# blindopen/TSM-Det-Pointcloud-

Measured on AMD Instinct MI355X. Metric: point-cloud frames/sec (fwd+bwd), higher is better.
Workload: dtype f32; 1 GPU; BASELINE configs[1]: KITTI-shaped synthetic, 20000 pts / 16000 active voxels per frame, full SECOND detector (VoxelBackBone8x) fwd+bwd+AdamW step; batch_per_gpu=4, global_batch=4, parallelism=dp1, voxelize_on_gpu=True

## Files before the change

include/spx.h:

```cpp
#ifndef SPX_H_
#define SPX_H_

#include <stddef.h>
#include <stdint.h>

#ifdef __cplusplus
extern "C" {
#endif

#define SPX_ABI_VERSION 3

#define SPX_OK 0
#define SPX_ERR_INVALID_ARG (-1)
#define SPX_ERR_WORKSPACE (-2)
#define SPX_ERR_UNSUPPORTED (-3)
#define SPX_ERR_LAUNCH (-4)
#define SPX_ERR_TOO_LARGE (-5)
#define SPX_ERR_CAPACITY (-7)
#define SPX_ERR_TABLE_FULL (-6)
#define SPX_ERR_RING_STALL (-8)
#define SPX_ERR_BATCH_STATS (-10)
#define SPX_ERR_OUT_OF_GRID (-9)

#define SPX_WS_PRECLEARED 1
// ... 112 lines not shown

int spx_bn_add_relu_fwd(const float *x, const float *res, int64_t n, const int64_t *d_n, int c, const float *gamma,
                        const float *beta, float *running_mean, float *running_var, int64_t *num_batches_tracked,
                        float momentum, float eps, int relu, float *y, int64_t y_ld, float *save_mean, float *save_invstd,
                        void *ws, size_t ws_bytes, spx_stream_t stream);
int spx_bn_add_relu_bwd(const float *x, const float *res, const float *dy, int64_t dy_ld, int64_t n, const int64_t *d_n,
                        int c, const float *gamma, const float *beta, const float *save_mean, const float *save_invstd, int relu,
                        float *dx, float *dres, float *dgamma, float *dbeta, void *ws, size_t ws_bytes,
                        spx_stream_t stream);

int spx_bn_apply(const float *x, const float *res, int64_t n, const int64_t *d_n, int c, const float *mean,
                 const float *invstd, const float *gamma, const float *beta, int relu, float *y, int64_t y_ld,
                 spx_stream_t stream);

int spx_bn_relu_fwd_from_sums(const float *x, int64_t n, const int64_t *d_n, int c, const float *partial, int64_t nblk,
                              const float *gamma,
                              const float *beta, float *running_mean, float *running_var, int64_t *num_batches_tracked,
                              float momentum, float eps, int relu, float *y, int64_t y_ld, float *save_mean,
                              float *save_invstd, spx_stream_t stream);

int64_t spx_wino_stat_rows(int32_t n, int32_t h, int32_t w);
int64_t spx_wino_weight_floats(int32_t cin, int32_t cout);
int spx_wino_weight(const float *w, int64_t s_o, int64_t s_i, int64_t s_a, int64_t s_b, int32_t cin, int32_t cout, int flip,
                    float *u, spx_stream_t stream);
int spx_conv2d_wino(const float *x, int64_t x_ld, const float *u, int32_t n, int32_t h, int32_t w, int32_t cin, int32_t cout,
                    const float *scale, const float *shift, int relu, float *y, int64_t y_ld, float *stat_partials,
                    spx_stream_t stream);

size_t spx_wino_wgrad_ws_bytes(int32_t cin, int32_t cout);
int spx_conv2d_wino_wgrad(const float *x, int64_t x_ld, const float *dy, int64_t dy_ld, int32_t n, int32_t h, int32_t w,
                          int32_t cin, int32_t cout, float *dw, int64_t s_o, int64_t s_i, int64_t s_a, int64_t s_b, void *ws,
                          size_t ws_bytes, spx_stream_t stream);

int spx_voxel_query(const float *new_xyz, const float *xyz, const int32_t *new_coords, const int32_t *point_indices,
                    int64_t m, int batch, const int32_t *shape3, int nsample, float radius, const int32_t *range3,
                    int32_t *idx, int32_t *cnt_unique, spx_stream_t stream);

int spx_voxel_query_dilated(const float *new_xyz, const float *xyz, const int32_t *new_coords,
                            const int32_t *point_indices, int64_t m, int batch, const int32_t *shape3, int nsample,
                            float former_radius, float radius, const int32_t *range3, const int32_t *stride3,
                            int32_t *idx, int32_t *cnt_unique, int32_t *idx_cnt, spx_stream_t stream);


size_t spx_furthest_point_sample_ws_bytes(int32_t b, int64_t n);
int spx_furthest_point_sample(const float *xyz, const float *weights, int32_t b, int64_t n, int32_t npoint, int32_t *idx,
                              void *ws, size_t ws_bytes, spx_stream_t stream);

size_t spx_furthest_point_sample_matrix_ws_bytes(int32_t b, int64_t n);
int spx_furthest_point_sample_matrix(const float *matrix, const float *weights, int32_t b, int64_t n, int32_t npoint,
                                     int32_t *idx, void *ws, size_t ws_bytes, spx_stream_t stream);

int spx_ball_query(const float *xyz, const float *new_xyz, int32_t b, int64_t n, int64_t m, float r_in, float r_out,
                   int32_t nsample, int32_t *idx_cnt, int32_t *idx, spx_stream_t stream);

int spx_group_points(const float *features, const int32_t *idx, int32_t b, int32_t c, int64_t n, int64_t m,
                     int32_t nsample, float *out, spx_stream_t stream);

size_t spx_group_points_bwd_ws_bytes(int32_t b, int64_t n, int64_t m, int32_t nsample);
int spx_group_points_bwd(const float *grad_out, const int32_t *idx, int32_t b, int32_t c, int64_t n, int64_t m,
                         int32_t nsample, float *grad_features, void *ws, size_t ws_bytes, spx_stream_t stream);

int spx_three_nn(const float *unknown, const float *known, int32_t b, int64_t n, int64_t m, float *dist2, int32_t *idx,
                 spx_stream_t stream);

int spx_three_interpolate(const float *features, const int32_t *idx, const float *weight, int32_t b, int32_t c, int64_t m,
                          int64_t n, float *out, spx_stream_t stream);
// ... 210 lines not shown
```

tsm-det-pointcloud-_amd/pcdet_amd/models/dense_heads/anchor_head_single.py:

```python
import os

import numpy as np
import torch
import torch.nn as nn
import torch.nn.functional as F

from ..model_utils import det_wgrad
from .anchor_head_template import AnchorHeadTemplate


_HYBRID = os.environ.get("SPX_HEAD_HYBRID", "1") != "0"


class _PointwiseHeadsFn(torch.autograd.Function):

    @staticmethod
    def forward(ctx, x, w, b):
        ctx.save_for_backward(x, w)
        return F.linear(x.permute(0, 2, 3, 1), w.flatten(1), b)

    @staticmethod
    def backward(ctx, dy):
        x, w = ctx.saved_tensors
        dy = dy.contiguous()
        n, h, wd, co = dy.shape
        dx = (dy.view(-1, co) @ w.flatten(1)).view(n, h, wd, x.shape[1]).permute(0, 3, 1, 2)
        if not dy.is_cuda:
            _, dw, db = torch.ops.aten.convolution_backward(dy.permute(0, 3, 1, 2), x, w, [co], [1, 1], [0, 0], [1, 1],
                                                            False, [0, 0], 1, [False, True, True])
            return dx, dw, db
        dw, db = det_wgrad.pointwise_wgrad(dy.view(-1, co), x.permute(0, 2, 3, 1).reshape(-1, x.shape[1]))
        return dx, dw.view_as(w), db


class AnchorHeadSingle(AnchorHeadTemplate):
    def __init__(self, model_cfg, input_channels, num_class, class_names, grid_size, point_cloud_range,
                 predict_boxes_when_training=True, **kwargs):
        super().__init__(model_cfg=model_cfg, num_class=num_class, class_names=class_names, grid_size=grid_size,
                         point_cloud_range=point_cloud_range, predict_boxes_when_training=predict_boxes_when_training)
        self.num_anchors_per_location = sum(self.num_anchors_per_location)
        self.conv_cls = nn.Conv2d(input_channels, self.num_anchors_per_location * self.num_class, kernel_size=1)
        self.conv_box = nn.Conv2d(input_channels, self.num_anchors_per_location * self.box_coder.code_size,
                                  kernel_size=1)
        if self.model_cfg.get('USE_DIRECTION_CLASSIFIER', None) is not None:
            self.conv_dir_cls = nn.Conv2d(input_channels, self.num_anchors_per_location * self.model_cfg.NUM_DIR_BINS,
                                          kernel_size=1)
        else:
            self.conv_dir_cls = None
        self.init_weights()

    def init_weights(self):
        pi = 0.01
        nn.init.constant_(self.conv_cls.bias, -np.log((1 - pi) / pi))
        nn.init.normal_(self.conv_box.weight, mean=0, std=0.001)

    def _heads(self, x):
        convs = [self.conv_cls, self.conv_box] + ([self.conv_dir_cls] if self.conv_dir_cls is not None else [])
        w = torch.cat([c.weight for c in convs], 0)
        b = torch.cat([c.bias for c in convs], 0)
        if (not x.is_contiguous(memory_format=torch.channels_last) or torch.is_autocast_enabled()
                or (torch.is_grad_enabled() and not _HYBRID)):
            y = F.conv2d(x, w, b).permute(0, 2, 3, 1)
        elif not torch.is_grad_enabled():
            y = F.linear(x.permute(0, 2, 3, 1), w.flatten(1), b)
        else:
            y = _PointwiseHeadsFn.apply(x, w, b)
        outs = [t.contiguous() for t in torch.split(y, [c.out_channels for c in convs], dim=3)]
        return outs[0], outs[1], (outs[2] if len(outs) > 2 else None)

    def forward(self, data_dict):
        if data_dict.get('encoded_bev_features', None) is not None:
            feats = data_dict['encoded_bev_features']
            x = feats[0] if len(feats) == 1 else torch.cat(feats, dim=1)
        else:
            x = data_dict['spatial_features_2d']
        x = x.float()
        cls_preds, box_preds, dir_cls_preds = self._heads(x)
        self.forward_ret_dict['cls_preds'] = cls_preds
        self.forward_ret_dict['box_preds'] = box_preds
        if dir_cls_preds is not None:
            self.forward_ret_dict['dir_cls_preds'] = dir_cls_preds
        if self.training:
            self.forward_ret_dict.update(self.assign_targets(gt_boxes=data_dict['gt_boxes']))
        if not self.training or self.predict_boxes_when_training:
            batch_cls_preds, batch_box_preds = self.generate_predicted_boxes(
                batch_size=data_dict['batch_size'], cls_preds=cls_preds, box_preds=box_preds,
                dir_cls_preds=dir_cls_preds)
            data_dict['batch_cls_preds'] = batch_cls_preds
            data_dict['batch_box_preds'] = batch_box_preds
            data_dict['cls_preds_normalized'] = False
        return data_dict
```

tsm-det-pointcloud-_amd/pcdet_amd/models/model_utils/det_wgrad.py:

```python
import torch
import torch.nn.functional as F

CHUNK = 4096


def mm_fixed(at, b):
    k = at.shape[1]
    s = k // CHUNK
    if s <= 1:
        return at @ b
    kk = s * CHUNK
    parts = torch.bmm(at[:, :kk].unflatten(1, (s, CHUNK)).transpose(0, 1), b[:kk].unflatten(0, (s, CHUNK)))
    out = parts.sum(0)
    if kk < k:
        out = out + at[:, kk:] @ b[kk:]
    return out


def rows_tn(a, b):
    return mm_fixed(a.t(), b)


def _rows(t):
    return t.permute(0, 2, 3, 1).reshape(-1, t.shape[1])


class _ConvFn(torch.autograd.Function):
    @staticmethod
    def forward(ctx, x, w, stride, padding, transposed):
        ctx.save_for_backward(x, w)
        ctx.cfg = (stride, padding, transposed)
        if transposed:
            return F.conv_transpose2d(x, w, None, stride)
        return F.conv2d(x, w, None, stride, padding)

    @staticmethod
    def backward(ctx, dy):
        x, w = ctx.saved_tensors
        stride, padding, transposed = ctx.cfg
        dx = dw = None
        if ctx.needs_input_grad[0]:
            dx = torch.ops.aten.convolution_backward(dy, x, w, None, [stride] * 2, [padding] * 2, [1, 1], transposed,
                                                     [0, 0], 1, [True, False, False])[0]
        if ctx.needs_input_grad[1]:
            n = x.shape[0]
            if transposed:
                s, co = stride, w.shape[1]
                h, wd = x.shape[2], x.shape[3]
                d = dy.permute(0, 2, 3, 1).reshape(n, h, s, wd, s, co).permute(0, 1, 3, 5, 2, 4).reshape(n * h * wd, co * s * s)
                dw = rows_tn(_rows(x), d).view_as(w)
            else:
                k, co = w.shape[2], w.shape[0]
                acc = None
                for i in range(n):
                    cols = F.unfold(x[i:i + 1], k, padding=padding, stride=stride)[0]
                    part = mm_fixed(cols, dy[i].permute(1, 2, 0).reshape(-1, co))
                    acc = part if acc is None else acc + part
                dw = acc.t().reshape(w.shape)
        return dx, dw, None, None, None


def usable(x, m):
    if not (x.is_cuda and x.dtype == torch.float32 and torch.is_grad_enabled() and m.weight.requires_grad
            and m.bias is None and m.groups == 1 and tuple(m.dilation) == (1, 1) and not torch.is_autocast_enabled()):
        return False
    k, s = tuple(m.kernel_size), tuple(m.stride)
    if k[0] != k[1] or s[0] != s[1]:
        return False
    if isinstance(m, torch.nn.ConvTranspose2d):
        return k == s and tuple(m.padding) == (0, 0) and tuple(m.output_padding) == (0, 0)
    return isinstance(m, torch.nn.Conv2d)


def conv2d(x, m, padding):
    return _ConvFn.apply(x, m.weight, int(m.stride[0]), int(padding), False)


def conv_transpose2d(x, m):
    return _ConvFn.apply(x, m.weight, int(m.stride[0]), 0, True)


def pointwise_wgrad(dy_rows, x_rows):
    return rows_tn(dy_rows, x_rows), dy_rows.sum(0)
```

tsm-det-pointcloud-_amd/spx/_lib.py:

```python
import ctypes
import os

import torch

_HERE = os.path.dirname(os.path.abspath(__file__))
LIB_PATH = os.environ.get("SPX_LIB_PATH") or os.path.join(os.path.dirname(_HERE), "csrc", "libspx.so")

SPX_ABI_VERSION = 3
SPX_MAX_KVOL = 32

_vp = ctypes.c_void_p
_i64 = ctypes.c_int64
_int = ctypes.c_int
_sz = ctypes.c_size_t
_i32p = ctypes.POINTER(ctypes.c_int32)
_f32p = ctypes.POINTER(ctypes.c_float)
_vpp = ctypes.POINTER(ctypes.c_void_p)

class PointMlp(ctypes.Structure):
    _fields_ = [("w1", _vp), ("bn_mean", _vp), ("bn_var", _vp), ("bn_weight", _vp), ("bn_bias", _vp),
                ("bn_eps", ctypes.c_float), ("w2", _vp), ("b2", _vp)]


_mlpp = ctypes.POINTER(PointMlp)
# ... 32 lines not shown
    "spx_conv_ring_stat_rows": (_int, []),
    "spx_conv_ring_tiles_per_wave": (_int, [_int]),
    "spx_conv_ring_plan": (_int, [_vp, _i64, _int, _i64, _vp, _vp, _vp]),
    "spx_conv_gemm_ring": (_int, [_vp, _i64, _int, _vp, _int, _int, _int, _vp, _i64, _i64, _vp, _vp, _vp, _int, _vp, _vp, _vp,
                                  _vp, _vp, _vp]),
    "spx_conv_wgrad_ws_bytes": (_sz, [_int, _int, _int, _i64]),
    "spx_conv_wgrad_counts_bytes": (_sz, [_int, _i64]),
    "spx_conv_wgrad_counts": (_int, [_vp, _i64, _int, _i64, _vp, _vp, _vp]),
    "spx_conv_wgrad": (_int, [_vp, _int, _vp, _int, _int, _vp, _i64, _i64, _vp, _vp, _vp, _vp, _sz, _vp]),
    "spx_densify": (_int, [_vp, _vp, _i64, _vp, _int, _int, _i32p, _int, _vp, _vp]),
    "spx_densify_bwd": (_int, [_vp, _vp, _i64, _vp, _int, _int, _i32p, _int, _vp, _vp]),
    "spx_boxes_iou_bev": (_int, [_vp, _i64, _vp, _i64, _int, _vp, _vp]),
    "spx_nms_ws_bytes": (_sz, [_i64]),
    "spx_nms_bev": (_int, [_vp, _i64, ctypes.c_float, _int, _vp, _vp, _vp, _sz, _vp]),
    "spx_assign_targets_ws_bytes": (_sz, [_int, _int, _int]),
    "spx_bn_relu_ws_bytes": (_sz, [_int]),
    "spx_bn_relu_fwd": (_int, [_vp, _i64, _vp, _int, _vp, _vp, _vp, _vp, ctypes.c_float, ctypes.c_float, _int, _vp, _vp,
                               _vp, _vp, _sz, _vp]),
    "spx_bn_relu_bwd": (_int, [_vp, _vp, _i64, _vp, _int, _vp, _vp, _vp, _vp, _int, _vp, _vp, _vp, _vp, _sz, _vp]),
    "spx_bn_add_relu_fwd": (_int, [_vp, _vp, _i64, _vp, _int, _vp, _vp, _vp, _vp, _vp, ctypes.c_float, ctypes.c_float, _int,
                                   _vp, _i64, _vp, _vp, _vp, _sz, _vp]),
    "spx_bn_add_relu_bwd": (_int, [_vp, _vp, _vp, _i64, _i64, _vp, _int, _vp, _vp, _vp, _vp, _int, _vp, _vp, _vp, _vp, _vp, _sz,
                                   _vp]),
    "spx_bn_apply": (_int, [_vp, _vp, _i64, _vp, _int, _vp, _vp, _vp, _vp, _int, _vp, _i64, _vp]),
    "spx_wino_weight_floats": (_i64, [_int, _int]),
    "spx_wino_weight": (_int, [_vp, _i64, _i64, _i64, _i64, _int, _int, _int, _vp, _vp]),
    "spx_conv2d_wino": (_int, [_vp, _i64, _vp, _int, _int, _int, _int, _int, _vp, _vp, _int, _vp, _i64, _vp, _vp]),
    "spx_wino_stat_rows": (_i64, [_int, _int, _int]),
    "spx_bn_relu_fwd_from_sums": (_int, [_vp, _i64, _vp, _int, _vp, _i64, _vp, _vp, _vp, _vp, _vp, ctypes.c_float, ctypes.c_float,
                                         _int, _vp, _i64, _vp, _vp, _vp]),
    "spx_wino_wgrad_ws_bytes": (_sz, [_int, _int]),
    "spx_conv2d_wino_wgrad": (_int, [_vp, _i64, _vp, _i64, _int, _int, _int, _int, _int, _vp, _i64, _i64, _i64, _i64, _vp, _sz,
                                     _vp]),
    "spx_anchor_loss_ws_bytes": (_sz, [_int, _i64]),
    "spx_anchor_loss": (_int, [_vp, _vp, _vp, _vp, _vp, _vp, _int, _i64, _int, _int, ctypes.c_float, ctypes.c_float,
                               ctypes.c_float, ctypes.c_float, ctypes.c_float, ctypes.c_float, _vp, _vp, _vp, _vp, _vp, _sz,
                               _vp]),
    "spx_assign_targets": (_int, [_vp, _int, _i64, _int, _vp, _int, _int, _vp, _int, _vp, _vp, _vp, _vp, _vp, _vp, _sz,
                                  _vp]),
    "spx_furthest_point_sample_ws_bytes": (_sz, [ctypes.c_int32, _i64]),
    "spx_furthest_point_sample": (_int, [_vp, _vp, ctypes.c_int32, _i64, ctypes.c_int32, _vp, _vp, _sz, _vp]),
    "spx_furthest_point_sample_matrix_ws_bytes": (_sz, [ctypes.c_int32, _i64]),
    "spx_furthest_point_sample_matrix": (_int, [_vp, _vp, ctypes.c_int32, _i64, ctypes.c_int32, _vp, _vp, _sz, _vp]),
    "spx_ball_query": (_int, [_vp, _vp, ctypes.c_int32, _i64, _i64, ctypes.c_float, ctypes.c_float, ctypes.c_int32, _vp,
                              _vp, _vp]),
    "spx_group_points": (_int, [_vp, _vp, ctypes.c_int32, ctypes.c_int32, _i64, _i64, ctypes.c_int32, _vp, _vp]),
    "spx_group_points_bwd_ws_bytes": (_sz, [ctypes.c_int32, _i64, _i64, ctypes.c_int32]),
    "spx_group_points_bwd": (_int, [_vp, _vp, ctypes.c_int32, ctypes.c_int32, _i64, _i64, ctypes.c_int32, _vp, _vp, _sz,
                                    _vp]),
    "spx_three_nn": (_int, [_vp, _vp, ctypes.c_int32, _i64, _i64, _vp, _vp, _vp]),
    "spx_three_interpolate": (_int, [_vp, _vp, _vp, ctypes.c_int32, ctypes.c_int32, _i64, _i64, _vp, _vp]),
    "spx_three_interpolate_bwd_ws_bytes": (_sz, [ctypes.c_int32, _i64, _i64]),
    "spx_three_interpolate_bwd": (_int, [_vp, _vp, _vp, ctypes.c_int32, ctypes.c_int32, _i64, _i64, _vp, _vp, _sz, _vp]),
    "spx_points_in_boxes": (_int, [_vp, _vp, ctypes.c_int32, _i64, _i64, _vp, _vp]),
    "spx_roiaware_pool3d_ws_bytes": (_sz, [_i64, _i64, ctypes.c_int32, ctypes.c_int32, ctypes.c_int32]),
    "spx_roiaware_pool3d_fwd": (_int, [_vp, _vp, _vp, _i64, _i64, ctypes.c_int32, ctypes.c_int32, ctypes.c_int32,
                                       ctypes.c_int32, ctypes.c_int32, ctypes.c_int32, _vp, _vp, _vp, _vp, _vp, _sz, _vp]),
    "spx_roiaware_pool3d_bwd": (_int, [_vp, _vp, _vp, _vp, _i64, _i64, ctypes.c_int32, ctypes.c_int32, ctypes.c_int32,
                                       ctypes.c_int32, ctypes.c_int32, _vp, _vp]),
    "spx_group_project": (_int, [_vp, _vp, _vp, _vp, _vp, _vp, ctypes.c_int32, _i64, ctypes.c_int32, _i64, ctypes.c_int32,
                                 _vp, _vp]),
    "spx_group_project_bwd_ws_bytes": (_sz, [ctypes.c_int32, _i64, ctypes.c_int32, _i64, ctypes.c_int32]),
    "spx_group_project_bwd": (_int, [_vp, _vp, _vp, _vp, _vp, ctypes.c_int32, _i64, ctypes.c_int32, _i64, ctypes.c_int32,
                                     _vp, _vp, _vp, _sz, _vp]),
    "spx_point_vote": (_int, [_vp, _vp, ctypes.c_int32, ctypes.c_int32, _i64, _i64, _i64, _mlpp, ctypes.c_int32, _f32p,
                              _vp, _vp]),
# ... 114 lines not shown
```

tsm-det-pointcloud-_amd/spx/functional.py:

```python
import os
import weakref

import torch

from . import ops


def _packed(weight, mode):
    if weight.is_cuda and torch.cuda.is_current_stream_capturing():
        if not torch.is_grad_enabled():
            holder = weight._base if weight._base is not None else weight
            hit = (getattr(holder, "_spx_packed", None) or {}).get(
                (mode, weight.data_ptr(), tuple(weight.shape), tuple(weight.stride())))
            if hit is not None and hit[0] == weight._version:
                return _graph_constant(weight, hit[1], lambda w, out, mode=mode: ops.pack_weight(w, mode, out=out))
        return ops.pack_weight(weight, mode)
    holder = weight._base if weight._base is not None else weight
    cache = getattr(holder, "_spx_packed", None)
    if cache is None:
        cache = {}
        try:
            holder._spx_packed = cache
        except AttributeError:
            return ops.pack_weight(weight, mode)
# ... 99 lines not shown
    for w, (fwd, bwd) in zip(ws, bank.views):
        geom = (w.data_ptr(), tuple(w.shape), tuple(w.stride()))
        try:
            w._spx_packed = {(0,) + geom: (w._version, fwd), (1,) + geom: (w._version, bwd)}
        except AttributeError:
            pass
    return True


_ASYNC_WGRAD = os.environ.get("SPX_ASYNC_WGRAD", "1") != "0"
_DEFER_JOIN = os.environ.get("SPX_WGRAD_DEFER_JOIN", "1") != "0"
_SIDE_STREAMS = {}


def _side_stream(device):
    s = _SIDE_STREAMS.get(device.index)
    if s is None:
        s = _SIDE_STREAMS[device.index] = torch.cuda.Stream(device=device)
    return s


_DEFERRED = set()


def _join_after_backward(main, side, keep):
    def _join():
        main.wait_stream(side)
        keep.clear()
        _DEFERRED.clear()
    torch.autograd.Variable._execution_engine.queue_callback(_join)


def _off_critical_path(fn, reads, weight):
    dev = reads[0].device
    main = torch.cuda.current_stream(dev)
    side = _side_stream(dev)
    side.wait_stream(main)
    with torch.cuda.stream(side):
        g = fn()
    g.record_stream(main)
    if (_nobody_reads_before_the_optimizer(weight) and id(weight) not in _DEFERRED
            and tuple(g.shape) == tuple(weight.shape) and g.stride() == weight.stride()):
        _DEFERRED.add(id(weight))
        _join_after_backward(main, side, list(reads))
    else:
        main.wait_stream(side)
    return g


def _nobody_reads_before_the_optimizer(weight):
    if not _DEFER_JOIN or not weight.is_leaf or weight.grad is not None or torch.cuda.is_current_stream_capturing():
        return False
    if getattr(weight, "_backward_hooks", None) or getattr(weight, "_post_accumulate_grad_hooks", None):
        return False
    dist = torch.distributed
    if dist.is_available() and dist.is_initialized():
        return bool(getattr(weight, "_spx_manual_reduce", False))
    return True


def _conv(src, wp, c_dst, kvol, pair, ld, n_dst, flip, scale, shift, relu, d_n, rb, want_stats=False):
    out = stats = None
    if rb is not None and src.is_cuda and n_dst > 0 and src.shape[0] > 0:
        if ops.ring_ok(src.shape[1], c_dst, n_dst, kvol):
            perm, table, tld, plan = ops.ring_plan_for(rb, pair, ld, kvol, n_dst, d_n)
            out = ops.conv_gemm_ring(src, wp, c_dst, kvol, table, tld, n_dst, plan, flip_k=flip, scale=scale, shift=shift,
                                     relu=relu, d_n_dst=d_n, perm=perm, want_stats=want_stats)
            if want_stats:
                out, stats = out
        elif ops.balanced_ok(src.shape[1], c_dst, n_dst, rb, pair):
            if ops.grouped_ok(rb, kvol):
                perm, grouped, plan = ops.grouped_plan_for(rb, pair, ld, kvol, n_dst, d_n)
                out = ops.conv_gemm_balanced(src, wp, c_dst, kvol, grouped, n_dst, n_dst, plan, flip_k=flip, scale=scale,
                                             shift=shift, relu=relu, d_n_dst=d_n, perm=perm)
            else:
                plan = ops.plan_for(rb, pair, ld, kvol, n_dst, d_n)
                out = ops.conv_gemm_balanced(src, wp, c_dst, kvol, pair, ld, n_dst, plan, flip_k=flip, scale=scale,
                                             shift=shift, relu=relu, d_n_dst=d_n)
    if out is None:
        out = ops.conv_gemm(src, wp, c_dst, kvol, pair, ld, n_dst, flip_k=flip, scale=scale, shift=shift, relu=relu,
# ... 335 lines not shown
```

tsm-det-pointcloud-_amd/spx/ops.py:

```python
import ctypes
import os

import torch

from . import _lib
from ._lib import check, f_arr, i3

_WS = {}


_raw_stream = getattr(torch._C, "_cuda_getCurrentRawStream", None)


def _stream_handle(device):
    if _raw_stream is not None:
        idx = device.index
        return _raw_stream(torch.cuda.current_device() if idx is None else idx)
    return torch.cuda.current_stream(device).cuda_stream


def _stream(t):
    return ctypes.c_void_p(_stream_handle(t.device))


# ... 685 lines not shown
        raise ValueError("weight image does not match Cin=%d, Cout=%d" % (cin, cout))
    part = None
    if stats:
        part = torch.empty((lib.spx_wino_stat_rows(n, h, w), 2, cout), dtype=torch.float32, device=x.device)
    check(lib.spx_conv2d_wino(_ptr(x), x_ld, _ptr(u), n, h, w, cin, cout, _ptr(scale), _ptr(shift), int(bool(relu)),
                              _ptr(out), y_ld, _ptr(part), _stream(x)), "spx_conv2d_wino")
    return (out, part) if stats else out


def wino_wgrad_ok(cin, cout, w):
    return cin % 128 == 0 and cout % 128 == 0 and (w + 1) // 2 >= 8


def conv2d_wino_wgrad(x, dy, like):
    _need_gpu(x, dy)
    lib = _lib.load()
    n, cin, h, w = (int(v) for v in x.shape)
    cout = int(dy.shape[1])
    x_ld, dy_ld = _cl_ld(x), _cl_ld(dy)
    if x_ld is None:
        x = x.contiguous(memory_format=torch.channels_last)
        x_ld = _cl_ld(x)
    if dy_ld is None:
        dy = dy.contiguous(memory_format=torch.channels_last)
        dy_ld = _cl_ld(dy)
    assert tuple(like.shape) == (cout, cin, 3, 3) and tuple(dy.shape) == (n, cout, h, w)
    dw = torch.empty_like(like)
    so, si, sa, sb = dw.stride()
    wsb = lib.spx_wino_wgrad_ws_bytes(cin, cout)
    ws = workspace(x.device, wsb)
    check(lib.spx_conv2d_wino_wgrad(_ptr(x), x_ld, _ptr(dy), dy_ld, n, h, w, cin, cout, _ptr(dw), so, si, sa, sb, _ptr(ws), wsb,
                                    _stream(x)), "spx_conv2d_wino_wgrad")
    return dw


def _cl_ld(t):
    if t.dtype != torch.float32 or t.dim() != 4:
        return None
    n, c, h, w = t.shape
    sn, sc, sh, sw = t.stride()
    ld = sw if w > 1 else (sh if h > 1 else c)
    if c > 1 and sc != 1:
        return None
    if ld < c or ld % 4 or t.data_ptr() % 16:
        return None
    if (w > 1 and sw != ld) or (h > 1 and sh != w * ld) or (n > 1 and sn != h * w * ld):
        return None
    return int(ld)


def bn_relu_bwd(x, dy, gamma, beta, mean, invstd, relu, residual=None, d_n=None):
    _need_gpu(x, dy)
    lib = _lib.load()
    n, c = x.shape
    if not _row_view_ok(dy, n, c):
        dy = dy.contiguous()
    dy_ld = dy.stride(0) if n > 1 else c
    dx = torch.empty_like(x)
    dres = torch.empty_like(x) if residual is not None else None
    dgamma = torch.empty((c,), dtype=torch.float32, device=x.device)
    dbeta = torch.empty((c,), dtype=torch.float32, device=x.device)
    if n == 0:
        out = (dx, dgamma.zero_(), dbeta.zero_())
        return out if residual is None else out + (dres,)
    wsb = lib.spx_bn_relu_ws_bytes(c)
    ws = workspace(x.device, wsb)
# ... 1232 lines not shown
```

Measured before the change: 294.6 frames/s.

## Add MFMA rows-wgrad kernel for pointwise heads, conv and deconv weight grads

Adds a new HIP kernel that computes weight gradients as split-K row reductions using fp32 MFMA 32x32x2 with double-buffered LDS and buffer loads, then a finalize kernel that sums slab partials and scatters results into per-segment weight and bias tensors. The anchor head passes the separate cls/box/dir weights and biases through, so the gradients land directly in each parameter without a cat and split. Conv and transposed-conv weight grads can also route to the kernel via tap and shuffle addressing. Weight-grad work runs on a side stream that joins after backward, aiming to remove rocBLAS/unfold overhead and copies, at the cost of a large partial-sum workspace and an extra reduction pass.

After: 294.5 frames/s, median of 2. No clear change (-0.0%).

```diff
diff --git a/include/spx.h b/include/spx.h
--- a/include/spx.h
+++ b/include/spx.h
@@ -168,6 +168,15 @@
                           int32_t cin, int32_t cout, float *dw, int64_t s_o, int64_t s_i, int64_t s_a, int64_t s_b, void *ws,
                           size_t ws_bytes, spx_stream_t stream);
 
+#define SPX_ROWS_POINTWISE 0
+#define SPX_ROWS_SHUFFLE 1
+#define SPX_ROWS_TAPS 2
+size_t spx_rows_wgrad_ws_bytes(int32_t m, int32_t n, int32_t k, int64_t rows, int64_t rows_per_slab);
+int spx_rows_wgrad(int32_t mode, const float *a, int64_t a_ld, int32_t m, const float *b, int64_t b_ld, int32_t n, int32_t batch,
+                   int32_t h, int32_t w, int32_t k, int32_t stride, int32_t pad, float *const *dw, float *const *db,
+                   const int32_t *seg_rows, int32_t n_seg, int64_t s_m, int64_t s_n, int64_t s_a, int64_t s_b,
+                   int64_t rows_per_slab, void *ws, size_t ws_bytes, spx_stream_t stream);
+
 int spx_voxel_query(const float *new_xyz, const float *xyz, const int32_t *new_coords, const int32_t *point_indices,
                     int64_t m, int batch, const int32_t *shape3, int nsample, float radius, const int32_t *range3,
                     int32_t *idx, int32_t *cnt_unique, spx_stream_t stream);
diff --git a/tsm-det-pointcloud-_amd/csrc/rows_wgrad.hip b/tsm-det-pointcloud-_amd/csrc/rows_wgrad.hip
--- /dev/null
+++ b/tsm-det-pointcloud-_amd/csrc/rows_wgrad.hip
@@ -0,0 +1,320 @@
+#include "spx_common.h"
+
+namespace {
+
+typedef float f32x16 __attribute__((ext_vector_type(16)));
+typedef float f32x4 __attribute__((ext_vector_type(4)));
+typedef float f32x2 __attribute__((ext_vector_type(2)));
+
+constexpr int kStepRows = 8;
+constexpr int kBlk = 128;
+constexpr int kThreads = 256;
+constexpr int kTargetWgs = 512;
+constexpr int kMinSlabRows = 64;
+constexpr int kMaxSeg = 4;
+constexpr int kMaxK = 7;
+constexpr uint32_t kOob = 0xFFFFFFF0u;
+
+struct Operand {
+  const float* p;
+  uint32_t bytes;
+  uint32_t ld4;
+  int32_t c;
+  int32_t h, w;
+  int32_t s;
+  int32_t use_g;
+  int32_t pad;
+};
+
+struct RowsArgs {
+  Operand a, b;
+  float* part;
+  float* colpart;
+  int64_t rows;
+  int64_t rows_per_slab;
+  int32_t hb, wb;
+  int32_t n_slab, kk, g, tiles_m, tiles_n;
+};
+
+__device__ __forceinline__ uint32_t row_offset(const Operand& o, int cn, int cy, int cx, int oy, int ox, bool ok, uint32_t chan4) {
+  const int yy = o.s * cy + oy, xx = o.s * cx + ox;
+  ok = ok && (unsigned)yy < (unsigned)o.h && (unsigned)xx < (unsigned)o.w;
+  return ok ? (((uint32_t)cn * (uint32_t)o.h + (uint32_t)yy) * (uint32_t)o.w + (uint32_t)xx) * o.ld4 + chan4 : kOob;
+}
+
+__global__ void __launch_bounds__(kThreads) k_rows_wgrad(RowsArgs a) {
+  __shared__ __attribute__((aligned(16))) float smem[2 * 2 * kStepRows * kBlk];
+  constexpr int kBufFloats = kStepRows * kBlk;
+  float* const as = smem;
+  float* const bs = smem + 2 * kBufFloats;
+
+  const int tid = threadIdx.x;
+  const int lane = tid & 63;
+  const int wave = __builtin_amdgcn_readfirstlane(tid >> 6);
+  const int l31 = lane & 31, lh = lane >> 5;
+
+  const int n_tile = a.tiles_m * a.tiles_n * a.g;
+  const int bid = blockIdx.x;
+  const int slab = (bid & 7) | ((bid / (8 * n_tile)) << 3);
+  if (slab >= a.n_slab) return;
+  int tile = (bid >> 3) % n_tile;
+  const int g = tile / (a.tiles_m * a.tiles_n);
+  tile -= g * (a.tiles_m * a.tiles_n);
+  const int mt = tile / a.tiles_n, nt = tile - mt * a.tiles_n;
+  const int ga = g / a.kk, gb = g - ga * a.kk;
+
+  const int64_t p_begin = (int64_t)slab * a.rows_per_slab;
+  int64_t p_end = p_begin + a.rows_per_slab;
+  if (p_end > a.rows) p_end = a.rows;
+  const int nsteps = (int)((p_end - p_begin + kStepRows - 1) / kStepRows);
+
+  const __amdgpu_buffer_rsrc_t rs_a = __builtin_amdgcn_make_buffer_rsrc(const_cast<float*>(a.a.p), 0, (int)a.a.bytes, 0x00020000);
+  const __amdgpu_buffer_rsrc_t rs_b = __builtin_amdgcn_make_buffer_rsrc(const_cast<float*>(a.b.p), 0, (int)a.b.bytes, 0x00020000);
+
+  const int lr = tid >> 5, lq = tid & 31;
+  const int cha = mt * kBlk + lq * 4, chb = nt * kBlk + lq * 4;
+  const bool cha_ok = cha < a.a.c, chb_ok = chb < a.b.c;
+  const int oya = a.a.use_g ? ga - a.a.pad : 0, oxa = a.a.use_g ? gb - a.a.pad : 0;
+  const int oyb = a.b.use_g ? ga - a.b.pad : 0, oxb = a.b.use_g ? gb - a.b.pad : 0;
+  int64_t p = p_begin + lr;
+  int cx = (int)(p % a.wb), cy = (int)((p / a.wb) % a.hb), cn = (int)(p / ((int64_t)a.wb * a.hb));
+  f32x4 ra, rb;
+  f32x4 csum = {0.f, 0.f, 0.f, 0.f};
+  auto issue_loads = [&]() {
+    const bool pv = p < p_end;
+    const uint32_t va = row_offset(a.a, cn, cy, cx, oya, oxa, pv && cha_ok, (uint32_t)cha * 4u);
+    const uint32_t vb = row_offset(a.b, cn, cy, cx, oyb, oxb, pv && chb_ok, (uint32_t)chb * 4u);
+    ra = __builtin_bit_cast(f32x4, __builtin_amdgcn_raw_buffer_load_b128(rs_a, (int)va, 0, 0));
+    rb = __builtin_bit_cast(f32x4, __builtin_amdgcn_raw_buffer_load_b128(rs_b, (int)vb, 0, 0));
+    p += kStepRows;
+    cx += kStepRows;
+    while (cx >= a.wb) {
+      cx -= a.wb;
+      if (++cy >= a.hb) {
+        cy = 0;
+        ++cn;
+      }
+    }
+  };
+  float* const a_dst = as + lr * kBlk + lq * 4;
+  float* const b_dst = bs + lr * kBlk + lq * 4;
+  auto store_lds = [&](int buf) {
+    *reinterpret_cast<f32x4*>(a_dst + buf * kBufFloats) = ra;
+    *reinterpret_cast<f32x4*>(b_dst + buf * kBufFloats) = rb;
+    csum += ra;
+  };
+
+  const int wm = wave & 1, wn = wave >> 1;
+  const float* const a_src = as + lh * kBlk + wm * 64 + l31 * 2;
+  const float* const b_src = bs + lh * kBlk + wn * 64 + l31 * 2;
+  f32x16 acc[2][2];
+#pragma unroll
+  for (int e = 0; e < 2; ++e)
+#pragma unroll
+    for (int f = 0; f < 2; ++f)
+#pragma unroll
+      for (int r = 0; r < 16; ++r) acc[e][f][r] = 0.f;
+  auto mma = [&](int buf) {
+    const float* pa = a_src + buf * kBufFloats;
+    const float* pb = b_src + buf * kBufFloats;
+    f32x2 av[4], bv[4];
+#pragma unroll
+    for (int q = 0; q < 4; ++q) {
+      av[q] = *reinterpret_cast<const f32x2*>(pa + q * 2 * kBlk);
+      bv[q] = *reinterpret_cast<const f32x2*>(pb + q * 2 * kBlk);
+    }
+#pragma unroll
+    for (int q = 0; q < 4; ++q) {
+#pragma unroll
+      for (int e = 0; e < 2; ++e)
+#pragma unroll
+        for (int f = 0; f < 2; ++f) acc[e][f] = __builtin_amdgcn_mfma_f32_32x32x2f32(av[q][e], bv[q][f], acc[e][f], 0, 0, 0);
+      if (q == 1) store_lds(buf ^ 1);
+      if (q == 2) issue_loads();
+    }
+  };
+
+  issue_loads();
+  store_lds(0);
+  issue_loads();
+  __syncthreads();
+  for (int s = 0; s < nsteps; ++s) {
+    mma(s & 1);
+    __syncthreads();
+  }
+
+  const int m_total = a.a.c, n_total = a.b.c;
+  {
+    const int m0 = mt * kBlk + wm * 64, n0 = nt * kBlk + wn * 64 + 2 * l31;
+    float* const out = a.part + ((int64_t)slab * a.g + g) * m_total * (int64_t)n_total;
+    if (n0 < n_total) {
+#pragma unroll
+      for (int e = 0; e < 2; ++e)
+#pragma unroll
+        for (int r = 0; r < 16; ++r) {
+          const int m = m0 + 2 * ((r & 3) + 8 * (r >> 2) + 4 * lh) + e;
+          if (m < m_total) {
+            const f32x2 v = {acc[e][0][r], acc[e][1][r]};
+            *reinterpret_cast<f32x2*>(out + (int64_t)m * n_total + n0) = v;
+          }
+        }
+    }
+  }
+
+  if (a.colpart != nullptr && nt == 0 && g == 0) {
+    *reinterpret_cast<f32x4*>(smem + lr * kBlk + lq * 4) = csum;
+    __syncthreads();
+    if (tid < kBlk) {
+      float s = 0.f;
+#pragma unroll
+      for (int r = 0; r < kStepRows; ++r) s += smem[r * kBlk + tid];
+      const int m = mt * kBlk + tid;
+      if (m < m_total) a.colpart[(int64_t)slab * m_total + m] = s;
+    }
+  }
+}
+
+struct FinalArgs {
+  const float* part;
+  const float* colpart;
+  float* dw[kMaxSeg];
+  float* db[kMaxSeg];
+  int32_t seg_end[kMaxSeg];
+  int64_t s_m, s_n, s_a, s_b;
+  int32_t n_seg, n_slab, m, n, g, kk;
+  int32_t want_db;
+};
+
+__global__ void __launch_bounds__(256) k_rows_wgrad_final(FinalArgs f) {
+  const int64_t plane = (int64_t)f.m * f.n;
+  const int64_t total = plane * f.g;
+  const int64_t idx = (int64_t)blockIdx.x * 256 + threadIdx.x;
+  if (idx < total) {
+    const int n = (int)(idx % f.n);
+    const int m = (int)((idx / f.n) % f.m);
+    const int g = (int)(idx / plane);
+    const float* src = f.part + idx;
+    float s = 0.f;
+#pragma unroll 8
+    for (int k = 0; k < f.n_slab; ++k) s += src[(int64_t)k * total];
+    int seg = 0;
+    while (seg + 1 < f.n_seg && m >= f.seg_end[seg]) ++seg;
+    const int mb = seg ? f.seg_end[seg - 1] : 0;
+    const int ga = g / f.kk, gb = g - ga * f.kk;
+    f.dw[seg][(int64_t)(m - mb) * f.s_m + (int64_t)n * f.s_n + ga * f.s_a + gb * f.s_b] = s;
+    return;
+  }
+  const int64_t first_db = (total + 255) / 256 * 256;
+  const int64_t m = idx - first_db;
+  if (f.want_db && m >= 0 && m < f.m) {
+    float s = 0.f;
+#pragma unroll 8
+    for (int k = 0; k < f.n_slab; ++k) s += f.colpart[(int64_t)k * f.m + m];
+    int seg = 0;
+    while (seg + 1 < f.n_seg && m >= f.seg_end[seg]) ++seg;
+    const int mb = seg ? f.seg_end[seg - 1] : 0;
+    f.db[seg][m - mb] = s;
+  }
+}
+
+static int64_t slab_rows(int32_t m, int32_t n, int32_t k, int64_t rows, int64_t rows_per_slab) {
+  if (rows_per_slab > 0) return rows_per_slab;
+  const int64_t tiles = (int64_t)((m + kBlk - 1) / kBlk) * ((n + kBlk - 1) / kBlk) * k * k;
+  int64_t s = kTargetWgs / tiles;
+  if (s < 1) s = 1;
+  int64_t per = ((rows + s - 1) / s + kStepRows - 1) / kStepRows * kStepRows;
+  return per < kMinSlabRows ? kMinSlabRows : per;
+}
+
+static bool shape_ok(int32_t m, int32_t n, int32_t k, int64_t rows) {
+  return m > 0 && n > 0 && k >= 1 && k <= kMaxK && rows > 0 && (m & 3) == 0 && (n & 3) == 0;
+}
+
+}
+
+extern "C" size_t spx_rows_wgrad_ws_bytes(int32_t m, int32_t n, int32_t k, int64_t rows, int64_t rows_per_slab) {
+  if (!shape_ok(m, n, k, rows) || rows_per_slab < 0) return 0;
+  const int64_t per = slab_rows(m, n, k, rows, rows_per_slab);
+  const int64_t ns = (rows + per - 1) / per;
+  return spx_align((size_t)ns * k * k * (size_t)m * n * sizeof(float)) + spx_align((size_t)ns * m * sizeof(float));
+}
+
+extern "C" int spx_rows_wgrad(int32_t mode, const float* a, int64_t a_ld, int32_t m, const float* b, int64_t b_ld, int32_t n,
+                              int32_t batch, int32_t h, int32_t w, int32_t k, int32_t stride, int32_t pad, float* const* dw,
+                              float* const* db, const int32_t* seg_rows, int32_t n_seg, int64_t s_m, int64_t s_n, int64_t s_a,
+                              int64_t s_b, int64_t rows_per_slab, void* ws, size_t ws_bytes, spx_stream_t stream) {
+  if (a == nullptr || b == nullptr || dw == nullptr || seg_rows == nullptr || batch <= 0 || h <= 0 || w <= 0 || m <= 0 ||
+      n <= 0 || k <= 0 || stride <= 0 || pad < 0 || rows_per_slab < 0 || n_seg <= 0 || a_ld < m || b_ld < n)
+    return SPX_ERR_INVALID_ARG;
+  if (mode < SPX_ROWS_POINTWISE || mode > SPX_ROWS_TAPS || n_seg > kMaxSeg || k > kMaxK || (m & 3) || (n & 3) || (a_ld & 3) ||
+      (b_ld & 3) || ((uintptr_t)a & 15) || ((uintptr_t)b & 15))
+    return SPX_ERR_UNSUPPORTED;
+  if ((mode == SPX_ROWS_POINTWISE && (k != 1 || stride != 1 || pad != 0)) || (mode == SPX_ROWS_SHUFFLE && (k != stride || pad != 0)) ||
+      (mode != SPX_ROWS_POINTWISE && db != nullptr) || pad >= k)
+    return SPX_ERR_UNSUPPORTED;
+  int32_t seg_sum = 0;
+  for (int i = 0; i < n_seg; ++i) {
+    if (seg_rows[i] <= 0 || dw[i] == nullptr || (db != nullptr && db[i] == nullptr)) return SPX_ERR_INVALID_ARG;
+    seg_sum += seg_rows[i];
+  }
+  if (seg_sum != m) return SPX_ERR_INVALID_ARG;
+
+  int32_t ha = h, wa = w, hb = h, wb = w, gh = h, gw = w;
+  if (mode == SPX_ROWS_SHUFFLE) {
+    hb = h * stride;
+    wb = w * stride;
+  } else if (mode == SPX_ROWS_TAPS) {
+    if (h + 2 * pad < k || w + 2 * pad < k) return SPX_ERR_INVALID_ARG;
+    gh = hb = (h + 2 * pad - k) / stride + 1;
+    gw = wb = (w + 2 * pad - k) / stride + 1;
+  }
+  const int64_t rows = (int64_t)batch * gh * gw;
+  const int64_t a_bytes = ((int64_t)batch * ha * wa - 1) * a_ld * 4 + (int64_t)m * 4;
+  const int64_t b_bytes = ((int64_t)batch * hb * wb - 1) * b_ld * 4 + (int64_t)n * 4;
+  if (a_bytes >= 0xFFFFFFF0ll || b_bytes >= 0xFFFFFFF0ll || rows >= 0x7FFFFFFFll) return SPX_ERR_TOO_LARGE;
+  if (ws == nullptr || ws_bytes < spx_rows_wgrad_ws_bytes(m, n, k, rows, rows_per_slab)) return SPX_ERR_WORKSPACE;
+
+  const int64_t per = slab_rows(m, n, k, rows, rows_per_slab);
+  const int64_t ns = (rows + per - 1) / per;
+  RowsArgs r;
+  r.a = Operand{a, (uint32_t)a_bytes, (uint32_t)a_ld * 4u, m, ha, wa, mode == SPX_ROWS_TAPS ? stride : 1, mode == SPX_ROWS_TAPS, pad};
+  r.b = Operand{b, (uint32_t)b_bytes, (uint32_t)b_ld * 4u, n, hb, wb, mode == SPX_ROWS_SHUFFLE ? stride : 1,
+                mode == SPX_ROWS_SHUFFLE, 0};
+  r.part = static_cast<float*>(ws);
+  r.colpart = db != nullptr
+                  ? reinterpret_cast<float*>(static_cast<char*>(ws) + spx_align((size_t)ns * k * k * (size_t)m * n * sizeof(float)))
+                  : nullptr;
+  r.rows = rows;
+  r.rows_per_slab = per;
+  r.hb = gh;
+  r.wb = gw;
+  r.n_slab = (int32_t)ns;
+  r.kk = k;
+  r.g = k * k;
+  r.tiles_m = (m + kBlk - 1) / kBlk;
+  r.tiles_n = (n + kBlk - 1) / kBlk;
+  const int64_t n_tile = (int64_t)r.tiles_m * r.tiles_n * r.g;
+  const int64_t grid = (ns + 7) / 8 * 8 * n_tile;
+  const int64_t total = (int64_t)r.g * m * n;
+  const int64_t fgrid = (total + 255) / 256 + (db != nullptr ? (m + 255) / 256 : 0);
+  if (grid >= 0x7FFFFFFFll || fgrid >= 0x7FFFFFFFll) return SPX_ERR_TOO_LARGE;
+  hipLaunchKernelGGL(k_rows_wgrad, dim3((unsigned)grid), dim3(kThreads), 0, spx_s(stream), r);
+  SPX_CHECK_LAUNCH();
+
+  FinalArgs f;
+  f.part = r.part;
+  f.colpart = r.colpart;
+  int32_t end = 0;
+  for (int i = 0; i < kMaxSeg; ++i) {
+    f.dw[i] = i < n_seg ? dw[i] : nullptr;
+    f.db[i] = (i < n_seg && db != nullptr) ? db[i] : nullptr;
+    if (i < n_seg) end += seg_rows[i];
+    f.seg_end[i] = end;
+  }
+  f.s_m = s_m; f.s_n = s_n; f.s_a = s_a; f.s_b = s_b;
+  f.n_seg = n_seg; f.n_slab = (int32_t)ns; f.m = m; f.n = n; f.g = r.g; f.kk = k;
+  f.want_db = db != nullptr;
+  hipLaunchKernelGGL(k_rows_wgrad_final, dim3((unsigned)fgrid), dim3(256), 0, spx_s(stream), f);
+  SPX_CHECK_LAUNCH();
+  return SPX_OK;
+}
diff --git a/tsm-det-pointcloud-_amd/pcdet_amd/models/dense_heads/anchor_head_single.py b/tsm-det-pointcloud-_amd/pcdet_amd/models/dense_heads/anchor_head_single.py
--- a/tsm-det-pointcloud-_amd/pcdet_amd/models/dense_heads/anchor_head_single.py
+++ b/tsm-det-pointcloud-_amd/pcdet_amd/models/dense_heads/anchor_head_single.py
@@ -15,22 +15,28 @@
 class _PointwiseHeadsFn(torch.autograd.Function):
 
     @staticmethod
-    def forward(ctx, x, w, b):
-        ctx.save_for_backward(x, w)
+    def forward(ctx, x, *wb):
+        ws, bs = wb[0::2], wb[1::2]
+        w, b = (ws[0], bs[0]) if len(ws) == 1 else (torch.cat(ws, 0), torch.cat(bs, 0))
+        ctx.save_for_backward(x, w, *wb)
         return F.linear(x.permute(0, 2, 3, 1), w.flatten(1), b)
 
     @staticmethod
     def backward(ctx, dy):
-        x, w = ctx.saved_tensors
+        x, w = ctx.saved_tensors[:2]
+        wb = ctx.saved_tensors[2:]
+        ws, bs = wb[0::2], wb[1::2]
         dy = dy.contiguous()
         n, h, wd, co = dy.shape
         dx = (dy.view(-1, co) @ w.flatten(1)).view(n, h, wd, x.shape[1]).permute(0, 3, 1, 2)
+        sizes = [t.shape[0] for t in ws]
         if not dy.is_cuda:
             _, dw, db = torch.ops.aten.convolution_backward(dy.permute(0, 3, 1, 2), x, w, [co], [1, 1], [0, 0], [1, 1],
                                                             False, [0, 0], 1, [False, True, True])
-            return dx, dw, db
-        dw, db = det_wgrad.pointwise_wgrad(dy.view(-1, co), x.permute(0, 2, 3, 1).reshape(-1, x.shape[1]))
-        return dx, dw.view_as(w), db
+            dws, dbs = dw.split(sizes, 0), db.split(sizes, 0)
+        else:
+            dws, dbs = det_wgrad.pointwise_heads_wgrad(dy.view(-1, co), x.permute(0, 2, 3, 1).reshape(-1, x.shape[1]), ws, bs)
+        return (dx,) + tuple(t for pair in zip(dws, dbs) for t in pair)
 
 
 class AnchorHeadSingle(AnchorHeadTemplate):
@@ -56,15 +62,19 @@
 
     def _heads(self, x):
         convs = [self.conv_cls, self.conv_box] + ([self.conv_dir_cls] if self.conv_dir_cls is not None else [])
-        w = torch.cat([c.weight for c in convs], 0)
-        b = torch.cat([c.bias for c in convs], 0)
+        def cat():
+            return torch.cat([c.weight for c in convs], 0), torch.cat([c.bias for c in convs], 0)
         if (not x.is_contiguous(memory_format=torch.channels_last) or torch.is_autocast_enabled()
                 or (torch.is_grad_enabled() and not _HYBRID)):
+            w, b = cat()
             y = F.conv2d(x, w, b).permute(0, 2, 3, 1)
         elif not torch.is_grad_enabled():
+            w, b = cat()
             y = F.linear(x.permute(0, 2, 3, 1), w.flatten(1), b)
+        elif det_wgrad.NATIVE:
+            y = _PointwiseHeadsFn.apply(x, *[t for c in convs for t in (c.weight, c.bias)])
         else:
-            y = _PointwiseHeadsFn.apply(x, w, b)
+            y = _PointwiseHeadsFn.apply(x, *cat())
         outs = [t.contiguous() for t in torch.split(y, [c.out_channels for c in convs], dim=3)]
         return outs[0], outs[1], (outs[2] if len(outs) > 2 else None)
 
diff --git a/tsm-det-pointcloud-_amd/pcdet_amd/models/model_utils/det_wgrad.py b/tsm-det-pointcloud-_amd/pcdet_amd/models/model_utils/det_wgrad.py
--- a/tsm-det-pointcloud-_amd/pcdet_amd/models/model_utils/det_wgrad.py
+++ b/tsm-det-pointcloud-_amd/pcdet_amd/models/model_utils/det_wgrad.py
@@ -1,7 +1,13 @@
+import os
+
 import torch
 import torch.nn.functional as F
 
+from spx import functional as spxf
+from spx import ops
+
 CHUNK = 4096
+NATIVE = os.environ.get("SPX_TAIL_NATIVE_WGRAD", "0") != "0"
 
 
 def mm_fixed(at, b):
@@ -43,21 +49,39 @@
             dx = torch.ops.aten.convolution_backward(dy, x, w, None, [stride] * 2, [padding] * 2, [1, 1], transposed,
                                                      [0, 0], 1, [True, False, False])[0]
         if ctx.needs_input_grad[1]:
-            n = x.shape[0]
-            if transposed:
-                s, co = stride, w.shape[1]
-                h, wd = x.shape[2], x.shape[3]
-                d = dy.permute(0, 2, 3, 1).reshape(n, h, s, wd, s, co).permute(0, 1, 3, 5, 2, 4).reshape(n * h * wd, co * s * s)
-                dw = rows_tn(_rows(x), d).view_as(w)
+            if _native_ok(x, dy, w, padding, transposed):
+                if transposed:
+                    dw = _side(lambda: ops.conv_transpose2d_rows_wgrad(x, dy, w), [x, dy], w)
+                else:
+                    dw = _side(lambda: ops.conv2d_rows_wgrad(x, dy, w, stride, padding), [x, dy], w)
             else:
-                k, co = w.shape[2], w.shape[0]
-                acc = None
-                for i in range(n):
-                    cols = F.unfold(x[i:i + 1], k, padding=padding, stride=stride)[0]
-                    part = mm_fixed(cols, dy[i].permute(1, 2, 0).reshape(-1, co))
-                    acc = part if acc is None else acc + part
-                dw = acc.t().reshape(w.shape)
+                dw = _conv_wgrad_torch(x, w, dy, stride, padding, transposed)
         return dx, dw, None, None, None
+
+
+def _conv_wgrad_torch(x, w, dy, stride, padding, transposed):
+    n = x.shape[0]
+    if transposed:
+        s, co = stride, w.shape[1]
+        h, wd = x.shape[2], x.shape[3]
+        d = dy.permute(0, 2, 3, 1).reshape(n, h, s, wd, s, co).permute(0, 1, 3, 5, 2, 4).reshape(n * h * wd, co * s * s)
+        return rows_tn(_rows(x), d).view_as(w)
+    k, co = w.shape[2], w.shape[0]
+    acc = None
+    for i in range(n):
+        cols = F.unfold(x[i:i + 1], k, padding=padding, stride=stride)[0]
+        part = mm_fixed(cols, dy[i].permute(1, 2, 0).reshape(-1, co))
+        acc = part if acc is None else acc + part
+    return acc.t().reshape(w.shape)
+
+
+def _native_ok(x, dy, w, padding, transposed):
+    return (NATIVE and dy.is_cuda and x.is_cuda and x.dtype == dy.dtype == w.dtype == torch.float32 and w.shape[2] == w.shape[3]
+            and ops.rows_wgrad_ok(int(w.shape[0]), int(w.shape[1]), int(w.shape[2]), 0 if transposed else padding))
+
+
+def _side(fn, reads, weight):
+    return spxf._off_critical_path(fn, reads, weight) if spxf._ASYNC_WGRAD else fn()
 
 
 def usable(x, m):
@@ -82,3 +106,17 @@
 
 def pointwise_wgrad(dy_rows, x_rows):
     return rows_tn(dy_rows, x_rows), dy_rows.sum(0)
+
+
+def pointwise_heads_wgrad(dy_rows, x_rows, weights, biases):
+    co, ci = dy_rows.shape[1], x_rows.shape[1]
+    if (NATIVE and dy_rows.is_cuda and dy_rows.dtype == x_rows.dtype == torch.float32 and ops.rows_wgrad_ok(co, ci)
+            and all(t.dtype == torch.float32 for t in list(weights) + list(biases))):
+        def fn():
+            dws, dbs = ops.pointwise_rows_wgrad(dy_rows, x_rows, weights, biases)
+            return dws + dbs
+        gs = _side(fn, [dy_rows, x_rows], list(weights) + list(biases))
+        return gs[:len(weights)], gs[len(weights):]
+    dw, db = pointwise_wgrad(dy_rows, x_rows)
+    sizes = [t.shape[0] for t in weights]
+    return [g.reshape(t.shape) for g, t in zip(dw.split(sizes, 0), weights)], list(db.split(sizes, 0))
diff --git a/tsm-det-pointcloud-_amd/spx/_lib.py b/tsm-det-pointcloud-_amd/spx/_lib.py
--- a/tsm-det-pointcloud-_amd/spx/_lib.py
+++ b/tsm-det-pointcloud-_amd/spx/_lib.py
@@ -88,6 +88,9 @@
     "spx_wino_wgrad_ws_bytes": (_sz, [_int, _int]),
     "spx_conv2d_wino_wgrad": (_int, [_vp, _i64, _vp, _i64, _int, _int, _int, _int, _int, _vp, _i64, _i64, _i64, _i64, _vp, _sz,
                                      _vp]),
+    "spx_rows_wgrad_ws_bytes": (_sz, [_int, _int, _int, _i64, _i64]),
+    "spx_rows_wgrad": (_int, [_int, _vp, _i64, _int, _vp, _i64, _int, _int, _int, _int, _int, _int, _int, _vpp, _vpp, _i32p, _int,
+                              _i64, _i64, _i64, _i64, _i64, _vp, _sz, _vp]),
     "spx_anchor_loss_ws_bytes": (_sz, [_int, _i64]),
     "spx_anchor_loss": (_int, [_vp, _vp, _vp, _vp, _vp, _vp, _int, _i64, _int, _int, ctypes.c_float, ctypes.c_float,
                                ctypes.c_float, ctypes.c_float, ctypes.c_float, ctypes.c_float, _vp, _vp, _vp, _vp, _vp, _sz,
diff --git a/tsm-det-pointcloud-_amd/spx/functional.py b/tsm-det-pointcloud-_amd/spx/functional.py
--- a/tsm-det-pointcloud-_amd/spx/functional.py
+++ b/tsm-det-pointcloud-_amd/spx/functional.py
@@ -155,6 +155,8 @@
 
 
 def _off_critical_path(fn, reads, weight):
+    if isinstance(weight, (list, tuple)):
+        return _off_critical_path_many(fn, reads, list(weight))
     dev = reads[0].device
     main = torch.cuda.current_stream(dev)
     side = _side_stream(dev)
@@ -169,6 +171,24 @@
     else:
         main.wait_stream(side)
     return g
+
+
+def _off_critical_path_many(fn, reads, weights):
+    dev = reads[0].device
+    main = torch.cuda.current_stream(dev)
+    side = _side_stream(dev)
+    side.wait_stream(main)
+    with torch.cuda.stream(side):
+        gs = list(fn())
+    for g in gs:
+        g.record_stream(main)
+    if all(_nobody_reads_before_the_optimizer(w) and id(w) not in _DEFERRED and tuple(g.shape) == tuple(w.shape)
+           and g.stride() == w.stride() for g, w in zip(gs, weights)):
+        _DEFERRED.update(id(w) for w in weights)
+        _join_after_backward(main, side, list(reads))
+    else:
+        main.wait_stream(side)
+    return gs
 
 
 def _nobody_reads_before_the_optimizer(weight):
diff --git a/tsm-det-pointcloud-_amd/spx/ops.py b/tsm-det-pointcloud-_amd/spx/ops.py
--- a/tsm-det-pointcloud-_amd/spx/ops.py
+++ b/tsm-det-pointcloud-_amd/spx/ops.py
@@ -741,6 +741,87 @@
     check(lib.spx_conv2d_wino_wgrad(_ptr(x), x_ld, _ptr(dy), dy_ld, n, h, w, cin, cout, _ptr(dw), so, si, sa, sb, _ptr(ws), wsb,
                                     _stream(x)), "spx_conv2d_wino_wgrad")
     return dw
+
+
+ROWS_POINTWISE, ROWS_SHUFFLE, ROWS_TAPS = 0, 1, 2
+
+
+def rows_wgrad_ok(m, n, k=1, pad=0):
+    return m > 0 and n > 0 and m % 4 == 0 and n % 4 == 0 and 1 <= k <= 7 and 0 <= pad < k
+
+
+def _rows_ok(t, c):
+    return (t.dim() == 2 and t.dtype == torch.float32 and t.shape[1] == c and (t.shape[1] == 1 or t.stride(1) == 1)
+            and t.stride(0) >= c and t.stride(0) % 4 == 0 and t.data_ptr() % 16 == 0)
+
+
+def _rows_wgrad(mode, a, a_ld, m, b, b_ld, n, batch, h, w, k, stride, pad, rows, dws, dbs, strides, rows_per_slab):
+    lib = _lib.load()
+    wsb = lib.spx_rows_wgrad_ws_bytes(m, n, k, rows, rows_per_slab)
+    ws = workspace(a.device, wsb)
+    nseg = len(dws)
+    dwp = (ctypes.c_void_p * nseg)(*[t.data_ptr() for t in dws])
+    dbp = (ctypes.c_void_p * nseg)(*[t.data_ptr() for t in dbs]) if dbs is not None else None
+    seg = (ctypes.c_int32 * nseg)(*[int(t.shape[0]) for t in dws])
+    s_m, s_n, s_a, s_b = strides
+    check(lib.spx_rows_wgrad(mode, _ptr(a), a_ld, m, _ptr(b), b_ld, n, batch, h, w, k, stride, pad, dwp, dbp, seg, nseg, s_m, s_n,
+                             s_a, s_b, rows_per_slab, _ptr(ws), wsb, _stream(a)), "spx_rows_wgrad")
+
+
+def _cl_map(t):
+    ld = _cl_ld(t)
+    if ld is None:
+        t = t.contiguous(memory_format=torch.channels_last)
+        ld = _cl_ld(t)
+        if ld is None:
+            raise _lib.SpxError("spx_rows_wgrad: not a float32 map of a multiple of 4 channels")
+    return t, ld
+
+
+def conv2d_rows_wgrad(x, dy, like, stride, padding, rows_per_slab=0):
+    _need_gpu(x, dy)
+    n, cin, h, w = (int(v) for v in x.shape)
+    cout, k = int(like.shape[0]), int(like.shape[2])
+    ho, wo = (h + 2 * padding - k) // stride + 1, (w + 2 * padding - k) // stride + 1
+    assert tuple(like.shape) == (cout, cin, k, k) and tuple(dy.shape) == (n, cout, ho, wo)
+    x, x_ld = _cl_map(x)
+    dy, dy_ld = _cl_map(dy)
+    dw = torch.empty_like(like)
+    so, si, sa, sb = dw.stride()
+    _rows_wgrad(ROWS_TAPS, x, x_ld, cin, dy, dy_ld, cout, n, h, w, k, stride, padding, n * ho * wo, [dw.permute(1, 0, 2, 3)],
+                None, (si, so, sa, sb), rows_per_slab)
+    return dw
+
+
+def conv_transpose2d_rows_wgrad(x, dy, like, rows_per_slab=0):
+    _need_gpu(x, dy)
+    n, cin, h, w = (int(v) for v in x.shape)
+    cout, k = int(like.shape[1]), int(like.shape[2])
+    assert tuple(like.shape) == (cin, cout, k, k) and tuple(dy.shape) == (n, cout, k * h, k * w)
+    x, x_ld = _cl_map(x)
+    dy, dy_ld = _cl_map(dy)
+    dw = torch.empty_like(like)
+    si, so, sa, sb = dw.stride()
+    _rows_wgrad(ROWS_SHUFFLE, x, x_ld, cin, dy, dy_ld, cout, n, h, w, k, k, 0, n * h * w, [dw], None, (si, so, sa, sb),
+                rows_per_slab)
+    return dw
+
+
+def pointwise_rows_wgrad(dy_rows, x_rows, likes_w, likes_b=None, rows_per_slab=0):
+    _need_gpu(dy_rows, x_rows)
+    p, co = (int(v) for v in dy_rows.shape)
+    ci = int(x_rows.shape[1])
+    if not _rows_ok(dy_rows, co):
+        dy_rows = dy_rows.contiguous()
+    if not _rows_ok(x_rows, ci):
+        x_rows = x_rows.contiguous()
+    assert x_rows.shape[0] == p and sum(int(t.shape[0]) for t in likes_w) == co
+    dws = [torch.empty_like(t) for t in likes_w]
+    assert all(d.shape[1] == ci and d.numel() == d.shape[0] * ci and d.stride(0) == ci and d.stride(1) == 1 for d in dws)
+    dbs = [torch.empty_like(t) for t in likes_b] if likes_b is not None else None
+    _rows_wgrad(ROWS_POINTWISE, dy_rows, dy_rows.stride(0), co, x_rows, x_rows.stride(0), ci, 1, 1, p, 1, 1, 0, p, dws, dbs,
+                (ci, 1, 0, 0), rows_per_slab)
+    return dws, dbs
 
 
 def _cl_ld(t):
```
